# rrwick/Filtlong

Measured on AMD Instinct MI355X. Metric: Mbases/s scored+sorted, higher is better.
Workload: dtype f64; 1 GPU; 10,000,000 synthetic reads per GPU x gamma(k=4) mean 10 kbp, Phred-only, --target_bases 50008889515 (50% of bases); C2; reads_total=10000000, bases_total=100017779031, window_size=250, parallelism=1 GPU, device=AMD Radeon Graphics (gfx950:sramecc+:xnack-), gpus_visible=1, cut=select

## Files before the change

filtlong_amd/csrc/flx_ctx.hip:

```cpp
#include <algorithm>
#include <cmath>
#include <numeric>

#include "flx_internal.h"
#include <vector>

static std::string g_create_error;

int flx_fail(flx_ctx *ctx, int code, const char *fmt, ...) {
    char buf[1024];
    va_list ap;
    va_start(ap, fmt);
    vsnprintf(buf, sizeof buf, fmt, ap);
    va_end(ap);
    if (ctx) ctx->err = buf;
    else g_create_error = buf;
    return code;
}

extern "C" int flx_abi_version(void) { return FLX_ABI_VERSION; }

extern "C" int flx_device_count(void) {
    int n = 0;
    if (hipGetDeviceCount(&n) != hipSuccess) return -1;
// ... 84 lines not shown
}

extern "C" void flx_ctx_destroy(flx_ctx *ctx) {
    if (!ctx) return;
    (void)hipSetDevice(ctx->device);
    (void)hipStreamSynchronize(ctx->stream);
    (void)flx_comm_destroy(ctx);
    for (auto &t : ctx->timed) {
        (void)hipEventDestroy(t.start);
        (void)hipEventDestroy(t.stop);
    }
    for (auto ev : ctx->event_pool) (void)hipEventDestroy(ev);
    if (ctx->d_lut_q) (void)hipFree(ctx->d_lut_q);
    if (ctx->d_lut_d) (void)hipFree(ctx->d_lut_d);
    if (ctx->scratch) (void)hipFree(ctx->scratch);
    if (ctx->pinned) (void)hipHostFree(ctx->pinned);
    for (void *w : ctx->ws)
        if (w) (void)hipFree(w);
    if (ctx->own_stream) (void)hipStreamDestroy(ctx->own_stream);
    delete ctx;
}

extern "C" int flx_ctx_set_stream(flx_ctx *ctx, void *hip_stream) {
    if (!ctx) return FLX_ERR_INVALID;
    ctx->stream = hip_stream ? (hipStream_t)hip_stream : ctx->own_stream;
    return FLX_OK;
}

extern "C" int flx_ctx_synchronize(flx_ctx *ctx) {
    if (!ctx) return FLX_ERR_INVALID;
// ... 161 lines not shown
```

filtlong_amd/csrc/flx_internal.h:

```cpp
#pragma once

#include <hip/hip_runtime.h>

#include <cstdarg>
#include <cstdint>
#include <cstdio>
#include <cstdlib>
#include <cstring>
#include <string>
#include <vector>

#include "../../include/filtlong_hip.h"

struct flx_comm;

struct flx_timed_launch {
    const char *name;
    hipEvent_t start, stop;
};

struct flx_ctx {
    int device = 0;
    hipStream_t own_stream = nullptr;
    hipStream_t stream = nullptr;
    hipDeviceProp_t prop;
    std::string err;
    bool last_kmer_fold_grid = false;
    const uint8_t *last_kmer_redo = nullptr;
    uint64_t last_kmer_redo_n = 0;
    const char *last_kmer_cover = "";
    bool last_kmer_locus = false;
    void *phred_pending = nullptr;
    const char *last_phred_kernel = "";

    double h_lut_q[257];
    double *d_lut_q = nullptr;
    double *d_lut_d = nullptr;
    int lut_d_ws = -1;

    flx_comm *comm = nullptr;

    bool timing = false;
    std::vector<flx_timed_launch> timed;
    std::vector<size_t> timed_open;
    std::vector<hipEvent_t> event_pool;

    void *scratch = nullptr;
    size_t scratch_bytes = 0;
// ... 66 lines not shown
```

filtlong_amd/csrc/score_phred.hip:

```cpp
#include <algorithm>

#include "flx_internal.h"
#include "score_phred_common.h"

using namespace flx_phred;

namespace {

#ifndef FLX_CH
#define FLX_CH 64
#endif
constexpr int CH = FLX_CH;
constexpr int PPR = CH / 16;

struct Fold {
    double s;
    double w;
    double mn;
};

__device__ __forceinline__ void head16(const double *lq, const uint32_t (&lw)[4], Fold &f) {
    double qj[16];
#pragma unroll
    for (int i = 0; i < 16; ++i) qj[i] = lds_f64(lq, lut_addr(lw[i >> 2], i & 3));
// ... 320 lines not shown
    a.redo_list = nullptr;
    a.use_private = nullptr;
    a.long_thr = 0x7fffffff;

    const long long n_slots = ((long long)p->window_size + CH - 1) / CH + 1;
    long long slots16 = n_slots * CH / 16 + 1;
    if ((slots16 & 1) == 0) slots16 += 1;
    const size_t ring_bytes = (size_t)64 * slots16 * 16;

    int waves = (int)((kLdsBudget - kLutBytes) / ring_bytes);
    const char *env = getenv("FLX_PHRED_KERNEL");
    const bool force_direct = env && strcmp(env, "direct") == 0;
    const bool force_ring = env && strcmp(env, "ring") == 0;
    const bool force_stream = env && strcmp(env, "stream") == 0;
    const bool force_dual = env && strcmp(env, "dual") == 0;
    PhredLong lp;
    FLX_CHECK(flx_phred_long_detect(ctx, a, plane_bytes, &lp));
    if (force_stream || force_dual) {
        FLX_CHECK(flx_phred_long_split(ctx, a, &lp));
        if (a.n_reads == 0) return FLX_OK;
        return force_stream ? flx_launch_score_phred_stream(ctx, a) : flx_launch_score_phred_dual(ctx, a);
    }
    if (!force_direct && !force_ring) {
        bool launched = false;
        a.n_slots = 0;
        a.stride = 0;
        FLX_CHECK(flx_launch_score_phred_regs(ctx, a, &launched, &lp));
        if (launched) return FLX_OK;
        FLX_CHECK(flx_phred_long_split(ctx, a, &lp));
        if (a.n_reads == 0) return FLX_OK;
        return flx_launch_score_phred_dual(ctx, a);
    }
// ... 54 lines not shown
```

filtlong_amd/csrc/score_phred_common.h:

```cpp
#pragma once

#include "flx_internal.h"

namespace flx_phred {

constexpr int LUT_PAD = 264;

struct PhredArgs {
    const uint8_t *plane;
    const uint64_t *offsets;
    const int32_t *lengths;
    const uint32_t *order;
    uint64_t n_reads;
    const double *lut_q;
    const double *lut_d;
    int ws;
    int n_slots;
    int stride;
    double ws_d;
    double clamp;
    flx_params p;
    double *mean_q;
    double *window_q;
    uint8_t *passed;
    unsigned int *ticket;
    unsigned int n_groups;
    unsigned int *redo_count;
    uint32_t *redo_list;
    const unsigned int *use_private;
    int long_thr;
};

__device__ __forceinline__ int wave_max(int v) {
#pragma unroll
    for (int o = 32; o > 0; o >>= 1) v = max(v, __shfl_xor(v, o, 64));
    return __builtin_amdgcn_readfirstlane(v);
}
__device__ __forceinline__ int wave_min(int v) {
#pragma unroll
    for (int o = 32; o > 0; o >>= 1) v = min(v, __shfl_xor(v, o, 64));
    return __builtin_amdgcn_readfirstlane(v);
}

__device__ __forceinline__ uint32_t byte_of(const uint4 &v, int i) {
    const uint32_t d = (i >> 2) == 0 ? v.x : (i >> 2) == 1 ? v.y : (i >> 2) == 2 ? v.z : v.w;
// ... 28 lines not shown
__device__ __forceinline__ void finish_read(const PhredArgs &a, uint32_t rid, int L, double s, double mn) {
    const double mean = 100.0 * s / (double)L;
    double window;
    if (L <= a.ws) window = mean;
    else {
        if (mn < a.clamp) mn = 0.0;
        window = 100.0 * mn;
    }
    a.mean_q[rid] = mean;
    a.window_q[rid] = window;
    a.passed[rid] = hard_cutoffs(a.p, L, mean, window);
}

constexpr int PHRED_LONG_NB = 13;
constexpr long long PHRED_LONG_FLOOR = 1 << 18;
struct PhredLong {
    bool on = false;
    bool fetched = false;
    bool done = false;
    bool forced = false;
    int t0 = 0;
    uint64_t plane_bytes = 0;
    unsigned long long *d_counts = nullptr;
    unsigned long long h_counts[3 * PHRED_LONG_NB] = {};
};

}

int flx_phred_long_detect(flx_ctx *ctx, const flx_phred::PhredArgs &a, uint64_t plane_bytes, flx_phred::PhredLong *lp);
long long flx_phred_long_threshold(const flx_ctx *ctx, const flx_phred::PhredLong *lp, int *b0);
int flx_phred_long_fetch(flx_ctx *ctx, flx_phred::PhredLong *lp);
int flx_phred_long_split(flx_ctx *ctx, flx_phred::PhredArgs &a, flx_phred::PhredLong *lp);

int flx_launch_score_phred_regs(flx_ctx *ctx, flx_phred::PhredArgs a, bool *launched, flx_phred::PhredLong *lp);
int flx_launch_score_phred_stream(flx_ctx *ctx, flx_phred::PhredArgs a);
int flx_launch_score_phred_dual(flx_ctx *ctx, flx_phred::PhredArgs a);
```

filtlong_amd/csrc/score_phred_long.hip:

```cpp
#include <algorithm>
#include <cerrno>
#include <chrono>

#include "flx_internal.h"
#include "fold_map.h"
#include "score_phred_common.h"

using namespace flx_phred;
using namespace flx_fold;

namespace {

constexpr int LANE_EL = 16;
constexpr int CHUNK = 64 * LANE_EL;
constexpr long long SAT = 1ll << 61;
constexpr long long NOSTEP = 1ll << 62;
constexpr long long M_LO = (1ll << 52) + 1, M_HI = (1ll << 53) - 1;
constexpr int SLOT_BLOCKS = 1024;
constexpr int MAX_OPEN = 16;
constexpr int MAX_STALL = 2;
constexpr int MIN_ADVANCE = 4;

__device__ __forceinline__ long long sat(long long x) { return x > SAT ? SAT : x < -SAT ? -SAT : x; }
__device__ __forceinline__ long long sel(bool c, long long x1, long long x0) { return x0 ^ ((x0 ^ x1) & -(long long)c); }

__device__ __forceinline__ Map2 compose_sat(const Map2 &a, const Map2 &b) {
    Map2 c;
    c.a0 = sat(a.a0 + sel((a.a0 & 1) != 0, b.a1, b.a0));
    c.a1 = sat(a.a1 + sel(((1 + a.a1) & 1) != 0, b.a1, b.a0));
// ... 121 lines not shown
    if (pos >= L) return make_uint4(0, 0, 0, 0);
    return *reinterpret_cast<const uint4 *>(q + pos);
}

__global__ void __launch_bounds__(256) flx_score_phred_long_find(const int32_t *lengths, uint64_t n, int ws, int t0, int nb,
                                                                 unsigned long long *out) {
    __shared__ unsigned long long sh[3 * PHRED_LONG_NB];
    for (int i = threadIdx.x; i < 3 * PHRED_LONG_NB; i += 256) sh[i] = 0;
    __syncthreads();
    const uint64_t stride = (uint64_t)gridDim.x * 256;
    for (uint64_t i0 = (uint64_t)blockIdx.x * 256 + threadIdx.x; i0 < n; i0 += 4 * stride) {
        int Ls[4];
#pragma unroll
        for (int u = 0; u < 4; ++u) Ls[u] = i0 + u * stride < n ? lengths[i0 + u * stride] : 0;
#pragma unroll
        for (int u = 0; u < 4; ++u) {
            const int L = Ls[u];
            if (L >= t0) {
                int b = 0;
                if (nb > 1) b = min(nb - 1, (31 - __clz(L)) - (31 - __clz(t0)));
                atomicAdd(&sh[b], 1ull);
                atomicAdd(&sh[PHRED_LONG_NB + b], (unsigned long long)((L + CHUNK - 1) / CHUNK));
                if (L > ws) atomicAdd(&sh[2 * PHRED_LONG_NB + b], (unsigned long long)((L - ws + CHUNK - 1) / CHUNK));
            }
        }
    }
    __syncthreads();
    for (int i = threadIdx.x; i < 3 * PHRED_LONG_NB; i += 256)
        if (sh[i]) atomicAdd(&out[i], sh[i]);
}

__global__ void __launch_bounds__(256) flx_score_phred_long_count(const int32_t *lengths, const uint32_t *order, uint64_t n,
                                                                  uint64_t per, int thr, uint32_t *blk) {
    const uint64_t s0 = (uint64_t)blockIdx.x * per, s1 = min(n, s0 + per);
    int c = 0;
    for (uint64_t t = s0; t < s1; t += 256) {
        const uint64_t slot = t + threadIdx.x;
        bool f = false;
        if (slot < s1) f = lengths[order ? order[slot] : (uint32_t)slot] >= thr;
        c += __syncthreads_count(f);
// ... 446 lines not shown
                    }
                    opened += stalled >= MAX_STALL ? MAX_OPEN : 1;
                    ls = fl + 1;
                }
                cs = f + 1;
            }
        }
    }
    if (lane == 0) finish_read(g.a, rid, L, S, mn);
}

size_t up256(size_t x) { return (x + 255) & ~(size_t)255; }

}

int flx_phred_long_detect(flx_ctx *ctx, const PhredArgs &a, uint64_t plane_bytes, PhredLong *lp) {
    *lp = PhredLong();
    lp->plane_bytes = plane_bytes;
    long long t0 = PHRED_LONG_FLOOR;
    const char *env = getenv("FLX_PHRED_LONG_MIN");
    if (env) {
        char *end = nullptr;
        errno = 0;
        const unsigned long long v = strtoull(env, &end, 10);
        if (!*env || *end || errno || env[0] == '-' || env[0] == '+' || env[0] == ' ')
            return flx_fail(ctx, FLX_ERR_INVALID, "FLX_PHRED_LONG_MIN=%s: expected a non-negative integer (bases)", env);
        if (v == 0 || v > 0x7fffffffull) return FLX_OK;
        t0 = (long long)v;
        lp->forced = true;
    }
    void *w;
    FLX_CHECK(flx_workspace(ctx, 3, 4096, &w));
    lp->d_counts = (unsigned long long *)w;
    lp->t0 = (int)t0;
    FLX_HIP(ctx, hipMemsetAsync(w, 0, sizeof lp->h_counts, ctx->stream));
    const unsigned grid = (unsigned)std::min<uint64_t>((a.n_reads + 255) / 256, 2048);
    hipLaunchKernelGGL(flx_score_phred_long_find, dim3(grid), dim3(256), 0, ctx->stream, a.lengths, a.n_reads, a.ws, (int)t0,
                       lp->forced ? 1 : PHRED_LONG_NB, lp->d_counts);
    FLX_HIP(ctx, hipGetLastError());
    lp->on = true;
    return FLX_OK;
}

int flx_phred_long_fetch(flx_ctx *ctx, PhredLong *lp) {
    if (!lp || !lp->on || lp->fetched) return FLX_OK;
    FLX_HIP(ctx, hipMemcpyAsync(lp->h_counts, lp->d_counts, sizeof lp->h_counts, hipMemcpyDeviceToHost, ctx->stream));
    lp->fetched = true;
    return FLX_OK;
}
// ... 114 lines not shown
```

filtlong_amd/csrc/score_phred_regs.hip:

```cpp
#include <algorithm>

#include "flx_internal.h"
#include "score_phred_common.h"

using namespace flx_phred;

#ifndef FLX_REGS_PART
#define FLX_REGS_PART 0
#endif

namespace {

template <bool PRIV>
struct Tab {
    static constexpr int ROW = PRIV ? 256 : 8;
    static constexpr int ENTRIES = PRIV ? 129 : LUT_PAD;
    static constexpr int BYTES = ROW * ENTRIES;
    static constexpr int QOFF = 0;
    static constexpr int DOFF = BYTES;
    static constexpr int ZIDX = PRIV ? 128 : 256;
    static constexpr int SLOT0 = 2 * BYTES;
};

template <bool PRIV, int SEL>
// ... 66 lines not shown
}

__device__ __forceinline__ void funnel(const uint32_t (&p0)[4], const uint32_t (&p1)[4], int fD, uint32_t fsh, uint32_t (&tw)[4]) {
    const uint32_t x[8] = {p0[0], p0[1], p0[2], p0[3], p1[0], p1[1], p1[2], p1[3]};
#define FLX_FUN(D) _Pragma("unroll") for (int d = 0; d < 4; ++d) tw[d] = __builtin_amdgcn_alignbyte(x[(D) + d + 1], x[(D) + d], fsh);
    switch (fD) {
        case 0: FLX_FUN(0) break;
        case 1: FLX_FUN(1) break;
        case 2: FLX_FUN(2) break;
        case 3: FLX_FUN(3) break;
        default: tw[0] = x[4]; tw[1] = x[5]; tw[2] = x[6]; tw[3] = x[7]; break;
    }
#undef FLX_FUN
}

template <int A, bool PRIV, int WAVES>
__global__ void __launch_bounds__(WAVES * 64) flx_score_phred_regs(const PhredArgs a) {
    using T = Tab<PRIV>;
    if (a.use_private && (*a.use_private != 0u) != PRIV) return;
    constexpr int R = ((A + 5 + 3) / 4) * 4;
    constexpr int RR = R / 4;
    constexpr int H = (A + 1 + 3) / 4;
    constexpr int SLOT_BYTES = 8192;
    static_assert(H <= RR, "prologue must fit one ring revolution");
    extern __shared__ __attribute__((aligned(16))) unsigned char smem[];

    if (PRIV) {
        for (int i = threadIdx.x; i < 129 * 32; i += WAVES * 64) {
            const int e = i >> 5;
            const double q = e < 128 ? a.lut_q[e] : 0.0, d = e < 128 ? a.lut_d[e] : 0.0;
            *reinterpret_cast<double *>(smem + T::QOFF + i * 8) = q;
            *reinterpret_cast<double *>(smem + T::DOFF + i * 8) = d;
        }
    } else {
        for (int i = threadIdx.x; i < 257; i += WAVES * 64) {
            *reinterpret_cast<double *>(smem + T::QOFF + i * 8) = a.lut_q[i];
            *reinterpret_cast<double *>(smem + T::DOFF + i * 8) = a.lut_d[i];
        }
    }
    __syncthreads();

    const int lane = threadIdx.x & 63;
    const int wave = threadIdx.x >> 6;
    unsigned char *slot = smem + T::SLOT0 + wave * SLOT_BYTES;
    const uint32_t slot_lds = (uint32_t)__builtin_amdgcn_readfirstlane((int)(T::SLOT0 + wave * SLOT_BYTES));
    const unsigned char *my_row = slot + lane * 64;
    const int rot = lane >> 2;
    const uint32_t laneoff = (uint32_t)(lane & 31) * 8u;
    const uint32_t zaddr = PRIV ? (uint32_t)(T::ZIDX * T::ROW) + laneoff : (uint32_t)(T::ZIDX * T::ROW);
    const int ws = a.ws;
    const int B = ws & 15;
    const int fD = (16 - B) >> 2;
    const uint32_t fsh = (uint32_t)(16 - B) & 3u;
    const double ws_d = a.ws_d;

  for (;;) {
    unsigned int group = 0;
    if (lane == 0) group = atomicAdd(a.ticket, 1u);
// ... 148 lines not shown
#pragma unroll
            for (int k = 0; k < 4; ++k) {
                const int t = 4 * sr + k;
                const int Tp = 4 * r + k;
                if (16 * Tp >= Lmax) break;
                steady_piece(ring[t], ring[(t + R - A - 1) % R], ring[(t + R - A) % R], Tp);
            }
        }
    }
done:
    if (live) {
        finish_read(a, rid, L, s, mn);
        if (PRIV && (bad & 0x80808080u)) a.redo_list[atomicAdd(a.redo_count, 1u)] = rid;
    }
  }
}

#if FLX_REGS_PART == 0
__global__ void __launch_bounds__(1024) flx_score_phred_stream(const PhredArgs a) {
    using T = Tab<false>;
    extern __shared__ __attribute__((aligned(16))) unsigned char smem[];
    for (int i = threadIdx.x; i < 257; i += 1024) {
        *reinterpret_cast<double *>(smem + T::QOFF + i * 8) = a.lut_q[i];
        *reinterpret_cast<double *>(smem + T::DOFF + i * 8) = a.lut_d[i];
    }
    __syncthreads();
    const int lane = threadIdx.x & 63;
    const uint32_t zaddr = (uint32_t)(T::ZIDX * T::ROW);
    const int ws = a.ws;
    const int A = ws >> 4, B = ws & 15;
// ... 253 lines not shown
                            }
                        }
                    }
                }
            }
#pragma unroll
            for (int k = 0; k < 4; ++k) {
                prev[k][0] = cur[k][0]; prev[k][1] = cur[k][1]; prev[k][2] = cur[k][2]; prev[k][3] = cur[k][3];
            }
        }
        asm volatile("s_waitcnt vmcnt(0)" ::: "memory");
        if (live) finish_read(a, rid, L, s, mn);
    }
}

__global__ void __launch_bounds__(256) flx_score_phred_redo(const PhredArgs a) {
    __shared__ double lq[LUT_PAD];
    __shared__ double ld[LUT_PAD];
    for (int i = threadIdx.x; i < 257; i += 256) {
        lq[i] = a.lut_q[i];
        ld[i] = a.lut_d[i];
    }
    __syncthreads();
    const unsigned int n = *a.redo_count;
    for (unsigned int i = blockIdx.x * 256 + threadIdx.x; i < n; i += gridDim.x * 256) {
        const uint32_t rid = a.redo_list[i];
        const int L = a.lengths[rid];
        const uint8_t *q = a.plane + a.offsets[rid];
        const int ws = a.ws;
        double s = 0.0, w = 0.0, mn = 0.0;
        const int head = L < ws ? L : ws;
        for (int j = 0; j < head; ++j) s += lq[q[j]];
        if (L > ws) {
// ... 1 lines not shown
            mn = w;
            for (int j = ws; j < L; ++j) {
                const uint32_t cj = q[j], ci = q[j - ws];
                s += lq[cj];
                w -= ld[ci];
                w += ld[cj];
                if (w < mn) mn = w;
            }
        }
        finish_read(a, rid, L, s, mn);
    }
}

#endif

template <int A, bool PRIV, int WAVES>
int launch_one(flx_ctx *ctx, PhredArgs &a) {
    using T = Tab<PRIV>;
    auto kern = flx_score_phred_regs<A, PRIV, WAVES>;
    const size_t lds = std::max<size_t>((size_t)T::SLOT0 + (size_t)WAVES * 8192, 84 * 1024);
    FLX_HIP(ctx, hipFuncSetAttribute((const void *)kern, hipFuncAttributeMaxDynamicSharedMemorySize, (int)lds));
    const uint64_t per_block = (uint64_t)WAVES;
    const unsigned grid = (unsigned)std::min<uint64_t>(((uint64_t)a.n_groups + per_block - 1) / per_block,
                                                       (uint64_t)ctx->prop.multiProcessorCount);
    if (!a.use_private) {
        ctx->last_phred_kernel = PRIV ? "flx_score_phred_regs_private" : "flx_score_phred_regs";
        flx_time_begin(ctx, ctx->last_phred_kernel);
    }
    hipLaunchKernelGGL(kern, dim3(grid), dim3(WAVES * 64), lds, ctx->stream, a);
    if (!a.use_private) flx_time_end(ctx);
    FLX_HIP(ctx, hipGetLastError());
    return FLX_OK;
}

template <int A, bool PRIV>
struct WavesFor {
    static constexpr int plain = A <= 7 ? 16 : A <= 15 ? 12 : 8;
    static constexpr int value = PRIV && plain > 11 ? 11 : plain;
};

template <int A>
int launch_a(flx_ctx *ctx, PhredArgs &a, bool priv) {
    if constexpr (A >= 32) {
        return launch_one<A, false, WavesFor<A, false>::value>(ctx, a);
    } else {
        return priv ? launch_one<A, true, WavesFor<A, true>::value>(ctx, a) : launch_one<A, false, WavesFor<A, false>::value>(ctx, a);
    }
}

}

#define FLX_REGS_CASE(AA) \
    case AA:              \
        *launched = true; \
        return launch_a<AA>(ctx, a, priv);
#define FLX_REGS_CAT2(a, b) a##b
#define FLX_REGS_CAT(a, b) FLX_REGS_CAT2(a, b)
#define FLX_REGS_WIDE_NAME FLX_REGS_CAT(flx_launch_score_phred_regs_part, FLX_REGS_PART)
#if FLX_REGS_PART == 0
int flx_launch_score_phred_regs_part0(flx_ctx *ctx, PhredArgs &a, bool priv, bool *launched) {
    switch (a.ws / 16) { FLX_REGS_CASE(0) FLX_REGS_CASE(1) FLX_REGS_CASE(2) FLX_REGS_CASE(3) FLX_REGS_CASE(4) FLX_REGS_CASE(5) FLX_REGS_CASE(6) FLX_REGS_CASE(7) default: return FLX_OK; }
}
#elif FLX_REGS_PART == 1
int flx_launch_score_phred_regs_part1(flx_ctx *ctx, PhredArgs &a, bool priv, bool *launched) {
    switch (a.ws / 16) { FLX_REGS_CASE(8) FLX_REGS_CASE(9) FLX_REGS_CASE(10) FLX_REGS_CASE(11) FLX_REGS_CASE(12) default: return FLX_OK; }
}
#elif FLX_REGS_PART == 2
int flx_launch_score_phred_regs_part2(flx_ctx *ctx, PhredArgs &a, bool priv, bool *launched) {
    switch (a.ws / 16) { FLX_REGS_CASE(13) FLX_REGS_CASE(14) FLX_REGS_CASE(15) FLX_REGS_CASE(16) FLX_REGS_CASE(17) default: return FLX_OK; }
}
#elif FLX_REGS_PART == 3
int flx_launch_score_phred_regs_part3(flx_ctx *ctx, PhredArgs &a, bool priv, bool *launched) {
    switch (a.ws / 16) { FLX_REGS_CASE(18) FLX_REGS_CASE(19) FLX_REGS_CASE(20) FLX_REGS_CASE(21) FLX_REGS_CASE(22) default: return FLX_OK; }
}
#elif FLX_REGS_PART == 4
int flx_launch_score_phred_regs_part4(flx_ctx *ctx, PhredArgs &a, bool priv, bool *launched) {
    switch (a.ws / 16) { FLX_REGS_CASE(23) FLX_REGS_CASE(24) FLX_REGS_CASE(25) FLX_REGS_CASE(26) FLX_REGS_CASE(27) default: return FLX_OK; }
}
#elif FLX_REGS_PART == 5
int flx_launch_score_phred_regs_part5(flx_ctx *ctx, PhredArgs &a, bool priv, bool *launched) {
    switch (a.ws / 16) { FLX_REGS_CASE(28) FLX_REGS_CASE(29) FLX_REGS_CASE(30) FLX_REGS_CASE(31) default: return FLX_OK; }
}
#else
int FLX_REGS_WIDE_NAME(flx_ctx *ctx, PhredArgs &a, bool priv, bool *launched) {
    constexpr int A0 = 32 + 4 * (FLX_REGS_PART - 6);
    switch (a.ws / 16) {
        FLX_REGS_CASE(A0) FLX_REGS_CASE(A0 + 1) FLX_REGS_CASE(A0 + 2)
#if FLX_REGS_PART < 7
        FLX_REGS_CASE(A0 + 3)
#endif
        default: return FLX_OK;
    }
}
#endif
#undef FLX_REGS_CASE

#if FLX_REGS_PART == 0
int flx_launch_score_phred_regs_part1(flx_ctx *ctx, PhredArgs &a, bool priv, bool *launched);
int flx_launch_score_phred_regs_part2(flx_ctx *ctx, PhredArgs &a, bool priv, bool *launched);
int flx_launch_score_phred_regs_part3(flx_ctx *ctx, PhredArgs &a, bool priv, bool *launched);
int flx_launch_score_phred_regs_part4(flx_ctx *ctx, PhredArgs &a, bool priv, bool *launched);
int flx_launch_score_phred_regs_part5(flx_ctx *ctx, PhredArgs &a, bool priv, bool *launched);
#define FLX_REGS_DECL(P) int flx_launch_score_phred_regs_part##P(flx_ctx *ctx, PhredArgs &a, bool priv, bool *launched);
FLX_REGS_DECL(6) FLX_REGS_DECL(7)
#undef FLX_REGS_DECL

namespace {
__global__ void __launch_bounds__(256) flx_phred_sample(const PhredArgs a, unsigned int *hist, unsigned int *done, unsigned int *use_private) {
    const uint64_t t = (uint64_t)blockIdx.x * 256 + threadIdx.x;
    uint64_t z = (t + 1) * 0x9E3779B97F4A7C15ULL;
    z = (z ^ (z >> 30)) * 0xBF58476D1CE4E5B9ULL;
    z = (z ^ (z >> 27)) * 0x94D049BB133111EBULL;
    z ^= z >> 31;
    const uint64_t r = z % a.n_reads;
    const int L = a.lengths[r];
    if (L > 0) {
        const uint32_t pos = (uint32_t)((z >> 32) % (uint64_t)L);
        atomicAdd(&hist[a.plane[a.offsets[r] + pos]], 1u);
    }
    __threadfence();
    __syncthreads();
    if (threadIdx.x != 0 || atomicAdd(done, 1u) != gridDim.x - 1) return;
    __threadfence();
    double tot = 0.0, conflicts = 0.0;
    bool high = false;
    for (int i = 0; i < 256; ++i) {
        const unsigned int h = __hip_atomic_load(&hist[i], __ATOMIC_RELAXED, __HIP_MEMORY_SCOPE_AGENT);
        tot += h;
        high = high || (i >= 128 && h != 0);
    }
    if (tot > 0) {
        for (int b = 0; b < 32; ++b) {
            double pb = 0.0, sq = 0.0;
            for (int e = b; e < 256; e += 32) {
                const double pe = __hip_atomic_load(&hist[e], __ATOMIC_RELAXED, __HIP_MEMORY_SCOPE_AGENT) / tot;
                pb += pe;
                sq += pe * pe;
            }
            conflicts += pb * pb - sq;
        }
    }
    *use_private = (!high && 496.0 * conflicts > 3.0) ? 1u : 0u;
}

struct PhredPending {
    PhredArgs a;
    PhredLong lp;
    bool chosen_on_device;
    long timed_index;
    const unsigned int *h_flag;
    const unsigned long long *h_counts;
};
}

int flx_launch_score_phred_stream(flx_ctx *ctx, PhredArgs a) {
    void *scr;
    FLX_CHECK(flx_scratch(ctx, 64, &scr));
// ... 23 lines not shown
    flx_time_begin(ctx, ctx->last_phred_kernel);
#define FLX_DUAL_LAUNCH(M)                                                                                                              \
    case M:                                                                                                                             \
        FLX_HIP(ctx, hipFuncSetAttribute((const void *)flx_score_phred_dual<M>, hipFuncAttributeMaxDynamicSharedMemorySize, (int)lds)); \
        hipLaunchKernelGGL(flx_score_phred_dual<M>, dim3(grid), dim3(DUAL_WAVES * 64), lds, ctx->stream, a);                            \
        break;
    switch ((a.ws >> 4) & 3) {
        FLX_DUAL_LAUNCH(0) FLX_DUAL_LAUNCH(1) FLX_DUAL_LAUNCH(2) FLX_DUAL_LAUNCH(3)
    }
#undef FLX_DUAL_LAUNCH
    flx_time_end(ctx);
    FLX_HIP(ctx, hipGetLastError());
    return FLX_OK;
}

int flx_launch_score_phred_regs(flx_ctx *ctx, PhredArgs a, bool *launched, PhredLong *lp) {
    *launched = false;
    const int A = a.ws / 16;
    if (A > 38) return FLX_OK;
    const char *env = getenv("FLX_PHRED_TABLES");
    bool priv = env && strcmp(env, "private") == 0;
    bool forced = env && (strcmp(env, "private") == 0 || strcmp(env, "plain") == 0);
    if (A >= 32) {
        forced = true;
        priv = false;
    }
    delete (PhredPending *)ctx->phred_pending;
    ctx->phred_pending = nullptr;
    void *scr;
    FLX_CHECK(flx_scratch(ctx, 2048 + a.n_reads * 4, &scr));
    void *pin;
    FLX_CHECK(flx_pinned(ctx, 1024, &pin));
    a.ticket = (unsigned int *)scr;
    a.redo_count = (unsigned int *)scr + 1;
    a.redo_list = (uint32_t *)((char *)scr + 2048);
    unsigned int *d_flag = (unsigned int *)scr + 3;
    FLX_HIP(ctx, hipMemsetAsync(scr, 0, 2048, ctx->stream));
    if (!forced) {
        hipLaunchKernelGGL(flx_phred_sample, dim3(64), dim3(256), 0, ctx->stream, a, (unsigned int *)((char *)scr + 64),
                           (unsigned int *)scr + 2, d_flag);
        a.use_private = d_flag;
    }
    a.long_thr = (int)std::min<long long>(flx_phred_long_threshold(ctx, lp, nullptr), 0x7fffffff);
    a.n_groups = (unsigned int)((a.n_reads + 63) / 64);
    auto part = [&](bool pv) -> int {
        if (A <= 7) return flx_launch_score_phred_regs_part0(ctx, a, pv, launched);
        if (A <= 12) return flx_launch_score_phred_regs_part1(ctx, a, pv, launched);
        if (A <= 17) return flx_launch_score_phred_regs_part2(ctx, a, pv, launched);
        if (A <= 22) return flx_launch_score_phred_regs_part3(ctx, a, pv, launched);
        if (A <= 27) return flx_launch_score_phred_regs_part4(ctx, a, pv, launched);
        if (A <= 31) return flx_launch_score_phred_regs_part5(ctx, a, pv, launched);
        typedef int (*part_fn)(flx_ctx *, PhredArgs &, bool, bool *);
        static const part_fn wide[2] = {flx_launch_score_phred_regs_part6, flx_launch_score_phred_regs_part7};
        return wide[(A - 32) / 4](ctx, a, false, launched);
    };
    long timed_index = -1;
    if (forced) {
        FLX_CHECK(part(priv));
    } else {
        ctx->last_phred_kernel = "flx_score_phred_regs";
        flx_time_scope t(ctx, ctx->last_phred_kernel);
        if (ctx->timing) timed_index = (long)ctx->timed.size() - 1;
        FLX_CHECK(part(false));
        FLX_CHECK(part(true));
    }
    if (!*launched) return FLX_OK;
    if (priv || !forced) {
        flx_time_begin(ctx, "flx_score_phred_redo");
        hipLaunchKernelGGL(flx_score_phred_redo, dim3(256), dim3(256), 0, ctx->stream, a);
        flx_time_end(ctx);
        FLX_HIP(ctx, hipGetLastError());
    }
    PhredPending *pd = new PhredPending();
    pd->a = a;
    pd->lp = *lp;
    pd->chosen_on_device = !forced;
    pd->timed_index = timed_index;
    pd->h_flag = (const unsigned int *)pin;
    pd->h_counts = (const unsigned long long *)((char *)pin + 64);
    ctx->phred_pending = pd;
    if (!forced) FLX_HIP(ctx, hipMemcpyAsync(pin, d_flag, 4, hipMemcpyDeviceToHost, ctx->stream));
    if (lp->on) FLX_HIP(ctx, hipMemcpyAsync((char *)pin + 64, lp->d_counts, sizeof lp->h_counts, hipMemcpyDeviceToHost, ctx->stream));
    lp->done = true;
    return FLX_OK;
}

int flx_phred_finish(flx_ctx *ctx) {
    PhredPending *pd = (PhredPending *)ctx->phred_pending;
    if (!pd) return FLX_OK;
    ctx->phred_pending = nullptr;
    struct Free {
        PhredPending *p;
        ~Free() { delete p; }
    } guard{pd};
    if (pd->chosen_on_device) {
        ctx->last_phred_kernel = *pd->h_flag ? "flx_score_phred_regs_private" : "flx_score_phred_regs";
        if (pd->timed_index >= 0 && (size_t)pd->timed_index < ctx->timed.size()) ctx->timed[pd->timed_index].name = ctx->last_phred_kernel;
// ... 13 lines not shown
```

Measured before the change: 3.331 million Mbases/s.

## Fuse phred sample and long-read detection into one prepare kernel, single regs launch

Merges the long-read length histogram and the table-conflict sampling into one prepare kernel. A persistent device state block, reset by the redo kernel, replaces the per-call memset. The plain and private score kernels, previously launched back to back with one exiting early, become a single kernel that branches on the device-side flag, and the sample's final reduction is parallelised. This removes several small launches and memsets per scoring call, at the cost of a wider block shape for the private variant and more template complexity.

```diff
diff --git a/filtlong_amd/csrc/flx_ctx.hip b/filtlong_amd/csrc/flx_ctx.hip
--- a/filtlong_amd/csrc/flx_ctx.hip
+++ b/filtlong_amd/csrc/flx_ctx.hip
@@ -122,6 +122,7 @@
     if (ctx->d_lut_q) (void)hipFree(ctx->d_lut_q);
     if (ctx->d_lut_d) (void)hipFree(ctx->d_lut_d);
     if (ctx->scratch) (void)hipFree(ctx->scratch);
+    if (ctx->phred_state) (void)hipFree(ctx->phred_state);
     if (ctx->pinned) (void)hipHostFree(ctx->pinned);
     for (void *w : ctx->ws)
         if (w) (void)hipFree(w);
diff --git a/filtlong_amd/csrc/flx_internal.h b/filtlong_amd/csrc/flx_internal.h
--- a/filtlong_amd/csrc/flx_internal.h
+++ b/filtlong_amd/csrc/flx_internal.h
@@ -32,6 +32,9 @@
     bool last_kmer_locus = false;
     void *phred_pending = nullptr;
     const char *last_phred_kernel = "";
+    void *phred_state = nullptr;
+    bool phred_state_clean = false;
+    hipStream_t phred_state_stream = nullptr;
 
     double h_lut_q[257];
     double *d_lut_q = nullptr;
diff --git a/filtlong_amd/csrc/score_phred.hip b/filtlong_amd/csrc/score_phred.hip
--- a/filtlong_amd/csrc/score_phred.hip
+++ b/filtlong_amd/csrc/score_phred.hip
@@ -358,8 +358,9 @@
     const bool force_ring = env && strcmp(env, "ring") == 0;
     const bool force_stream = env && strcmp(env, "stream") == 0;
     const bool force_dual = env && strcmp(env, "dual") == 0;
+    const bool regs_path = !force_stream && !force_dual && !force_direct && !force_ring && flx_phred_regs_serves(p->window_size);
     PhredLong lp;
-    FLX_CHECK(flx_phred_long_detect(ctx, a, plane_bytes, &lp));
+    FLX_CHECK(flx_phred_long_detect(ctx, a, plane_bytes, &lp, !regs_path));
     if (force_stream || force_dual) {
         FLX_CHECK(flx_phred_long_split(ctx, a, &lp));
         if (a.n_reads == 0) return FLX_OK;
diff --git a/filtlong_amd/csrc/score_phred_common.h b/filtlong_amd/csrc/score_phred_common.h
--- a/filtlong_amd/csrc/score_phred_common.h
+++ b/filtlong_amd/csrc/score_phred_common.h
@@ -28,7 +28,18 @@
     unsigned int *redo_count;
     uint32_t *redo_list;
     const unsigned int *use_private;
+    int force_private;
     int long_thr;
+};
+
+struct PhredState {
+    unsigned int ticket;
+    unsigned int redo_count;
+    unsigned int sample_done;
+    unsigned int use_private;
+    unsigned int pad[12];
+    unsigned int hist[256];
+    unsigned long long long_counts[3 * 13];
 };
 
 __device__ __forceinline__ int wave_max(int v) {
@@ -87,6 +98,18 @@
 
 constexpr int PHRED_LONG_NB = 13;
 constexpr long long PHRED_LONG_FLOOR = 1 << 18;
+constexpr int PHRED_LONG_CHUNK = 1024;
+static_assert(sizeof(PhredState::long_counts) == 3 * PHRED_LONG_NB * sizeof(unsigned long long), "PhredState holds the detection's counts");
+
+__device__ __forceinline__ void phred_long_count(int L, int ws, int t0, int nb, unsigned long long *sh) {
+    if (L < t0) return;
+    int b = 0;
+    if (nb > 1) b = min(nb - 1, (31 - __clz(L)) - (31 - __clz(t0)));
+    atomicAdd(&sh[b], 1ull);
+    atomicAdd(&sh[PHRED_LONG_NB + b], (unsigned long long)((L + PHRED_LONG_CHUNK - 1) / PHRED_LONG_CHUNK));
+    if (L > ws) atomicAdd(&sh[2 * PHRED_LONG_NB + b], (unsigned long long)((L - ws + PHRED_LONG_CHUNK - 1) / PHRED_LONG_CHUNK));
+}
+
 struct PhredLong {
     bool on = false;
     bool fetched = false;
@@ -100,11 +123,13 @@
 
 }
 
-int flx_phred_long_detect(flx_ctx *ctx, const flx_phred::PhredArgs &a, uint64_t plane_bytes, flx_phred::PhredLong *lp);
+int flx_phred_long_detect(flx_ctx *ctx, const flx_phred::PhredArgs &a, uint64_t plane_bytes, flx_phred::PhredLong *lp,
+                          bool count_now = true);
 long long flx_phred_long_threshold(const flx_ctx *ctx, const flx_phred::PhredLong *lp, int *b0);
 int flx_phred_long_fetch(flx_ctx *ctx, flx_phred::PhredLong *lp);
 int flx_phred_long_split(flx_ctx *ctx, flx_phred::PhredArgs &a, flx_phred::PhredLong *lp);
 
+bool flx_phred_regs_serves(int window_size);
 int flx_launch_score_phred_regs(flx_ctx *ctx, flx_phred::PhredArgs a, bool *launched, flx_phred::PhredLong *lp);
 int flx_launch_score_phred_stream(flx_ctx *ctx, flx_phred::PhredArgs a);
 int flx_launch_score_phred_dual(flx_ctx *ctx, flx_phred::PhredArgs a);
diff --git a/filtlong_amd/csrc/score_phred_long.hip b/filtlong_amd/csrc/score_phred_long.hip
--- a/filtlong_amd/csrc/score_phred_long.hip
+++ b/filtlong_amd/csrc/score_phred_long.hip
@@ -13,6 +13,7 @@
 
 constexpr int LANE_EL = 16;
 constexpr int CHUNK = 64 * LANE_EL;
+static_assert(CHUNK == PHRED_LONG_CHUNK, "the detection counts chunks of this size");
 constexpr long long SAT = 1ll << 61;
 constexpr long long NOSTEP = 1ll << 62;
 constexpr long long M_LO = (1ll << 52) + 1, M_HI = (1ll << 53) - 1;
@@ -164,16 +165,7 @@
 #pragma unroll
         for (int u = 0; u < 4; ++u) Ls[u] = i0 + u * stride < n ? lengths[i0 + u * stride] : 0;
 #pragma unroll
-        for (int u = 0; u < 4; ++u) {
-            const int L = Ls[u];
-            if (L >= t0) {
-                int b = 0;
-                if (nb > 1) b = min(nb - 1, (31 - __clz(L)) - (31 - __clz(t0)));
-                atomicAdd(&sh[b], 1ull);
-                atomicAdd(&sh[PHRED_LONG_NB + b], (unsigned long long)((L + CHUNK - 1) / CHUNK));
-                if (L > ws) atomicAdd(&sh[2 * PHRED_LONG_NB + b], (unsigned long long)((L - ws + CHUNK - 1) / CHUNK));
-            }
-        }
+        for (int u = 0; u < 4; ++u) phred_long_count(Ls[u], ws, t0, nb, sh);
     }
     __syncthreads();
     for (int i = threadIdx.x; i < 3 * PHRED_LONG_NB; i += 256)
@@ -650,7 +642,7 @@
 
 }
 
-int flx_phred_long_detect(flx_ctx *ctx, const PhredArgs &a, uint64_t plane_bytes, PhredLong *lp) {
+int flx_phred_long_detect(flx_ctx *ctx, const PhredArgs &a, uint64_t plane_bytes, PhredLong *lp, bool count_now) {
     *lp = PhredLong();
     lp->plane_bytes = plane_bytes;
     long long t0 = PHRED_LONG_FLOOR;
@@ -665,10 +657,14 @@
         t0 = (long long)v;
         lp->forced = true;
     }
+    lp->t0 = (int)t0;
+    if (!count_now) {
+        lp->on = true;
+        return FLX_OK;
+    }
     void *w;
     FLX_CHECK(flx_workspace(ctx, 3, 4096, &w));
     lp->d_counts = (unsigned long long *)w;
-    lp->t0 = (int)t0;
     FLX_HIP(ctx, hipMemsetAsync(w, 0, sizeof lp->h_counts, ctx->stream));
     const unsigned grid = (unsigned)std::min<uint64_t>((a.n_reads + 255) / 256, 2048);
     hipLaunchKernelGGL(flx_score_phred_long_find, dim3(grid), dim3(256), 0, ctx->stream, a.lengths, a.n_reads, a.ws, (int)t0,
diff --git a/filtlong_amd/csrc/score_phred_regs.hip b/filtlong_amd/csrc/score_phred_regs.hip
--- a/filtlong_amd/csrc/score_phred_regs.hip
+++ b/filtlong_amd/csrc/score_phred_regs.hip
@@ -104,10 +104,10 @@
 #undef FLX_FUN
 }
 
-template <int A, bool PRIV, int WAVES>
-__global__ void __launch_bounds__(WAVES * 64) flx_score_phred_regs(const PhredArgs a) {
+template <int A, bool PRIV, int WAVES, int BLOCK_WAVES>
+__device__ __forceinline__ void phred_regs_body(const PhredArgs &a) {
     using T = Tab<PRIV>;
-    if (a.use_private && (*a.use_private != 0u) != PRIV) return;
+    static_assert(WAVES <= BLOCK_WAVES, "a slot per scoring wave");
     constexpr int R = ((A + 5 + 3) / 4) * 4;
     constexpr int RR = R / 4;
     constexpr int H = (A + 1 + 3) / 4;
@@ -116,14 +116,14 @@
     extern __shared__ __attribute__((aligned(16))) unsigned char smem[];
 
     if (PRIV) {
-        for (int i = threadIdx.x; i < 129 * 32; i += WAVES * 64) {
+        for (int i = threadIdx.x; i < 129 * 32; i += BLOCK_WAVES * 64) {
             const int e = i >> 5;
             const double q = e < 128 ? a.lut_q[e] : 0.0, d = e < 128 ? a.lut_d[e] : 0.0;
             *reinterpret_cast<double *>(smem + T::QOFF + i * 8) = q;
             *reinterpret_cast<double *>(smem + T::DOFF + i * 8) = d;
         }
     } else {
-        for (int i = threadIdx.x; i < 257; i += WAVES * 64) {
+        for (int i = threadIdx.x; i < 257; i += BLOCK_WAVES * 64) {
             *reinterpret_cast<double *>(smem + T::QOFF + i * 8) = a.lut_q[i];
             *reinterpret_cast<double *>(smem + T::DOFF + i * 8) = a.lut_d[i];
         }
@@ -132,6 +132,7 @@
 
     const int lane = threadIdx.x & 63;
     const int wave = threadIdx.x >> 6;
+    if (WAVES < BLOCK_WAVES && wave >= WAVES) return;
     unsigned char *slot = smem + T::SLOT0 + wave * SLOT_BYTES;
     const uint32_t slot_lds = (uint32_t)__builtin_amdgcn_readfirstlane((int)(T::SLOT0 + wave * SLOT_BYTES));
     const unsigned char *my_row = slot + lane * 64;
@@ -310,6 +311,25 @@
         if (PRIV && (bad & 0x80808080u)) a.redo_list[atomicAdd(a.redo_count, 1u)] = rid;
     }
   }
+}
+
+template <int A, bool PRIV>
+struct WavesFor {
+    static constexpr int plain = A <= 7 ? 16 : A <= 15 ? 12 : 8;
+    static constexpr int value = PRIV && plain > 11 ? 11 : plain;
+};
+
+template <int A, bool BOTH>
+__global__ void __launch_bounds__((WavesFor<A, false>::value * 64)) flx_score_phred_regs(const PhredArgs a) {
+    constexpr int BW = WavesFor<A, false>::value;
+    if constexpr (BOTH) {
+        const bool priv = a.use_private ? *a.use_private != 0u : a.force_private != 0;
+        if (priv) {
+            phred_regs_body<A, true, WavesFor<A, true>::value, BW>(a);
+            return;
+        }
+    }
+    phred_regs_body<A, false, BW, BW>(a);
 }
 
 #if FLX_REGS_PART == 0
@@ -593,9 +613,14 @@
     }
 }
 
-__global__ void __launch_bounds__(256) flx_score_phred_redo(const PhredArgs a) {
+__global__ void __launch_bounds__(256) flx_score_phred_redo(const PhredArgs a, PhredState *st) {
     __shared__ double lq[LUT_PAD];
     __shared__ double ld[LUT_PAD];
+    if (blockIdx.x == 0) {
+        st->hist[threadIdx.x] = 0u;
+        if (threadIdx.x < 3 * PHRED_LONG_NB) st->long_counts[threadIdx.x] = 0ull;
+        if (threadIdx.x == 0) st->sample_done = 0u;
+    }
     for (int i = threadIdx.x; i < 257; i += 256) {
         lq[i] = a.lut_q[i];
         ld[i] = a.lut_d[i];
@@ -627,38 +652,21 @@
 
 #endif
 
-template <int A, bool PRIV, int WAVES>
-int launch_one(flx_ctx *ctx, PhredArgs &a) {
-    using T = Tab<PRIV>;
-    auto kern = flx_score_phred_regs<A, PRIV, WAVES>;
-    const size_t lds = std::max<size_t>((size_t)T::SLOT0 + (size_t)WAVES * 8192, 84 * 1024);
+template <int A>
+int launch_a(flx_ctx *ctx, PhredArgs &a) {
+    constexpr bool BOTH = A < 32;
+    constexpr int BW = WavesFor<A, false>::value;
+    auto kern = flx_score_phred_regs<A, BOTH>;
+    size_t lds = std::max<size_t>((size_t)Tab<false>::SLOT0 + (size_t)BW * 8192, 84 * 1024);
+    if (BOTH) lds = std::max<size_t>(lds, (size_t)Tab<true>::SLOT0 + (size_t)WavesFor<A, true>::value * 8192);
+    static_assert((size_t)Tab<true>::SLOT0 + 11 * 8192 <= 160 * 1024, "the bank-private tables and 11 slots fit the LDS");
     FLX_HIP(ctx, hipFuncSetAttribute((const void *)kern, hipFuncAttributeMaxDynamicSharedMemorySize, (int)lds));
-    const uint64_t per_block = (uint64_t)WAVES;
+    const uint64_t per_block = (uint64_t)BW;
     const unsigned grid = (unsigned)std::min<uint64_t>(((uint64_t)a.n_groups + per_block - 1) / per_block,
                                                        (uint64_t)ctx->prop.multiProcessorCount);
-    if (!a.use_private) {
-        ctx->last_phred_kernel = PRIV ? "flx_score_phred_regs_private" : "flx_score_phred_regs";
-        flx_time_begin(ctx, ctx->last_phred_kernel);
-    }
-    hipLaunchKernelGGL(kern, dim3(grid), dim3(WAVES * 64), lds, ctx->stream, a);
-    if (!a.use_private) flx_time_end(ctx);
+    hipLaunchKernelGGL(kern, dim3(grid), dim3(BW * 64), lds, ctx->stream, a);
     FLX_HIP(ctx, hipGetLastError());
     return FLX_OK;
-}
-
-template <int A, bool PRIV>
-struct WavesFor {
-    static constexpr int plain = A <= 7 ? 16 : A <= 15 ? 12 : 8;
-    static constexpr int value = PRIV && plain > 11 ? 11 : plain;
-};
-
-template <int A>
-int launch_a(flx_ctx *ctx, PhredArgs &a, bool priv) {
-    if constexpr (A >= 32) {
-        return launch_one<A, false, WavesFor<A, false>::value>(ctx, a);
-    } else {
-        return priv ? launch_one<A, true, WavesFor<A, true>::value>(ctx, a) : launch_one<A, false, WavesFor<A, false>::value>(ctx, a);
-    }
 }
 
 }
@@ -666,36 +674,36 @@
 #define FLX_REGS_CASE(AA) \
     case AA:              \
         *launched = true; \
-        return launch_a<AA>(ctx, a, priv);
+        return launch_a<AA>(ctx, a);
 #define FLX_REGS_CAT2(a, b) a##b
 #define FLX_REGS_CAT(a, b) FLX_REGS_CAT2(a, b)
 #define FLX_REGS_WIDE_NAME FLX_REGS_CAT(flx_launch_score_phred_regs_part, FLX_REGS_PART)
 #if FLX_REGS_PART == 0
-int flx_launch_score_phred_regs_part0(flx_ctx *ctx, PhredArgs &a, bool priv, bool *launched) {
+int flx_launch_score_phred_regs_part0(flx_ctx *ctx, PhredArgs &a, bool *launched) {
     switch (a.ws / 16) { FLX_REGS_CASE(0) FLX_REGS_CASE(1) FLX_REGS_CASE(2) FLX_REGS_CASE(3) FLX_REGS_CASE(4) FLX_REGS_CASE(5) FLX_REGS_CASE(6) FLX_REGS_CASE(7) default: return FLX_OK; }
 }
 #elif FLX_REGS_PART == 1
-int flx_launch_score_phred_regs_part1(flx_ctx *ctx, PhredArgs &a, bool priv, bool *launched) {
+int flx_launch_score_phred_regs_part1(flx_ctx *ctx, PhredArgs &a, bool *launched) {
     switch (a.ws / 16) { FLX_REGS_CASE(8) FLX_REGS_CASE(9) FLX_REGS_CASE(10) FLX_REGS_CASE(11) FLX_REGS_CASE(12) default: return FLX_OK; }
 }
 #elif FLX_REGS_PART == 2
-int flx_launch_score_phred_regs_part2(flx_ctx *ctx, PhredArgs &a, bool priv, bool *launched) {
+int flx_launch_score_phred_regs_part2(flx_ctx *ctx, PhredArgs &a, bool *launched) {
     switch (a.ws / 16) { FLX_REGS_CASE(13) FLX_REGS_CASE(14) FLX_REGS_CASE(15) FLX_REGS_CASE(16) FLX_REGS_CASE(17) default: return FLX_OK; }
 }
 #elif FLX_REGS_PART == 3
-int flx_launch_score_phred_regs_part3(flx_ctx *ctx, PhredArgs &a, bool priv, bool *launched) {
+int flx_launch_score_phred_regs_part3(flx_ctx *ctx, PhredArgs &a, bool *launched) {
     switch (a.ws / 16) { FLX_REGS_CASE(18) FLX_REGS_CASE(19) FLX_REGS_CASE(20) FLX_REGS_CASE(21) FLX_REGS_CASE(22) default: return FLX_OK; }
 }
 #elif FLX_REGS_PART == 4
-int flx_launch_score_phred_regs_part4(flx_ctx *ctx, PhredArgs &a, bool priv, bool *launched) {
+int flx_launch_score_phred_regs_part4(flx_ctx *ctx, PhredArgs &a, bool *launched) {
     switch (a.ws / 16) { FLX_REGS_CASE(23) FLX_REGS_CASE(24) FLX_REGS_CASE(25) FLX_REGS_CASE(26) FLX_REGS_CASE(27) default: return FLX_OK; }
 }
 #elif FLX_REGS_PART == 5
-int flx_launch_score_phred_regs_part5(flx_ctx *ctx, PhredArgs &a, bool priv, bool *launched) {
+int flx_launch_score_phred_regs_part5(flx_ctx *ctx, PhredArgs &a, bool *launched) {
     switch (a.ws / 16) { FLX_REGS_CASE(28) FLX_REGS_CASE(29) FLX_REGS_CASE(30) FLX_REGS_CASE(31) default: return FLX_OK; }
 }
 #else
-int FLX_REGS_WIDE_NAME(flx_ctx *ctx, PhredArgs &a, bool priv, bool *launched) {
+int FLX_REGS_WIDE_NAME(flx_ctx *ctx, PhredArgs &a, bool *launched) {
     constexpr int A0 = 32 + 4 * (FLX_REGS_PART - 6);
     switch (a.ws / 16) {
         FLX_REGS_CASE(A0) FLX_REGS_CASE(A0 + 1) FLX_REGS_CASE(A0 + 2)
@@ -709,17 +717,42 @@
 #undef FLX_REGS_CASE
 
 #if FLX_REGS_PART == 0
-int flx_launch_score_phred_regs_part1(flx_ctx *ctx, PhredArgs &a, bool priv, bool *launched);
-int flx_launch_score_phred_regs_part2(flx_ctx *ctx, PhredArgs &a, bool priv, bool *launched);
-int flx_launch_score_phred_regs_part3(flx_ctx *ctx, PhredArgs &a, bool priv, bool *launched);
-int flx_launch_score_phred_regs_part4(flx_ctx *ctx, PhredArgs &a, bool priv, bool *launched);
-int flx_launch_score_phred_regs_part5(flx_ctx *ctx, PhredArgs &a, bool priv, bool *launched);
-#define FLX_REGS_DECL(P) int flx_launch_score_phred_regs_part##P(flx_ctx *ctx, PhredArgs &a, bool priv, bool *launched);
+int flx_launch_score_phred_regs_part1(flx_ctx *ctx, PhredArgs &a, bool *launched);
+int flx_launch_score_phred_regs_part2(flx_ctx *ctx, PhredArgs &a, bool *launched);
+int flx_launch_score_phred_regs_part3(flx_ctx *ctx, PhredArgs &a, bool *launched);
+int flx_launch_score_phred_regs_part4(flx_ctx *ctx, PhredArgs &a, bool *launched);
+int flx_launch_score_phred_regs_part5(flx_ctx *ctx, PhredArgs &a, bool *launched);
+#define FLX_REGS_DECL(P) int flx_launch_score_phred_regs_part##P(flx_ctx *ctx, PhredArgs &a, bool *launched);
 FLX_REGS_DECL(6) FLX_REGS_DECL(7)
 #undef FLX_REGS_DECL
 
 namespace {
-__global__ void __launch_bounds__(256) flx_phred_sample(const PhredArgs a, unsigned int *hist, unsigned int *done, unsigned int *use_private) {
+constexpr int SAMPLE_WGS = 64;
+__global__ void __launch_bounds__(256) flx_phred_prepare(const PhredArgs a, PhredState *st, int do_sample, int long_t0, int long_nb) {
+    __shared__ unsigned long long sh[3 * PHRED_LONG_NB];
+    __shared__ unsigned int h[256];
+    __shared__ double cb[32];
+    __shared__ unsigned int last;
+    if (blockIdx.x == 0 && threadIdx.x == 0) {
+        st->ticket = 0u;
+        st->redo_count = 0u;
+    }
+    if (long_nb > 0) {
+        for (int i = threadIdx.x; i < 3 * PHRED_LONG_NB; i += 256) sh[i] = 0;
+        __syncthreads();
+        const uint64_t n = a.n_reads, stride = (uint64_t)gridDim.x * 256;
+        for (uint64_t i0 = (uint64_t)blockIdx.x * 256 + threadIdx.x; i0 < n; i0 += 4 * stride) {
+            int Ls[4];
+#pragma unroll
+            for (int u = 0; u < 4; ++u) Ls[u] = i0 + u * stride < n ? a.lengths[i0 + u * stride] : 0;
+#pragma unroll
+            for (int u = 0; u < 4; ++u) phred_long_count(Ls[u], a.ws, long_t0, long_nb, sh);
+        }
+        __syncthreads();
+        for (int i = threadIdx.x; i < 3 * PHRED_LONG_NB; i += 256)
+            if (sh[i]) atomicAdd(&st->long_counts[i], sh[i]);
+    }
+    if (!do_sample || blockIdx.x >= SAMPLE_WGS) return;
     const uint64_t t = (uint64_t)blockIdx.x * 256 + threadIdx.x;
     uint64_t z = (t + 1) * 0x9E3779B97F4A7C15ULL;
     z = (z ^ (z >> 30)) * 0xBF58476D1CE4E5B9ULL;
@@ -729,31 +762,34 @@
     const int L = a.lengths[r];
     if (L > 0) {
         const uint32_t pos = (uint32_t)((z >> 32) % (uint64_t)L);
-        atomicAdd(&hist[a.plane[a.offsets[r] + pos]], 1u);
+        atomicAdd(&st->hist[a.plane[a.offsets[r] + pos]], 1u);
     }
     __threadfence();
     __syncthreads();
-    if (threadIdx.x != 0 || atomicAdd(done, 1u) != gridDim.x - 1) return;
+    if (threadIdx.x == 0) last = atomicAdd(&st->sample_done, 1u) == SAMPLE_WGS - 1 ? 1u : 0u;
+    __syncthreads();
+    if (!last) return;
     __threadfence();
-    double tot = 0.0, conflicts = 0.0;
-    bool high = false;
-    for (int i = 0; i < 256; ++i) {
-        const unsigned int h = __hip_atomic_load(&hist[i], __ATOMIC_RELAXED, __HIP_MEMORY_SCOPE_AGENT);
-        tot += h;
-        high = high || (i >= 128 && h != 0);
-    }
-    if (tot > 0) {
-        for (int b = 0; b < 32; ++b) {
-            double pb = 0.0, sq = 0.0;
-            for (int e = b; e < 256; e += 32) {
-                const double pe = __hip_atomic_load(&hist[e], __ATOMIC_RELAXED, __HIP_MEMORY_SCOPE_AGENT) / tot;
+    h[threadIdx.x] = __hip_atomic_load(&st->hist[threadIdx.x], __ATOMIC_RELAXED, __HIP_MEMORY_SCOPE_AGENT);
+    const int high = __syncthreads_or(threadIdx.x >= 128 && h[threadIdx.x] != 0);
+    if (threadIdx.x < 32) {
+        double tot = 0.0;
+        for (int i = 0; i < 256; ++i) tot += h[i];
+        double pb = 0.0, sq = 0.0;
+        if (tot > 0) {
+            for (int e = threadIdx.x; e < 256; e += 32) {
+                const double pe = h[e] / tot;
                 pb += pe;
                 sq += pe * pe;
             }
-            conflicts += pb * pb - sq;
-        }
-    }
-    *use_private = (!high && 496.0 * conflicts > 3.0) ? 1u : 0u;
+        }
+        cb[threadIdx.x] = pb * pb - sq;
+    }
+    __syncthreads();
+    if (threadIdx.x != 0) return;
+    double conflicts = 0.0;
+    for (int b = 0; b < 32; ++b) conflicts += cb[b];
+    st->use_private = (!high && 496.0 * conflicts > 3.0) ? 1u : 0u;
 }
 
 struct PhredPending {
@@ -807,10 +843,12 @@
     return FLX_OK;
 }
 
+bool flx_phred_regs_serves(int window_size) { return window_size / 16 <= 38; }
+
 int flx_launch_score_phred_regs(flx_ctx *ctx, PhredArgs a, bool *launched, PhredLong *lp) {
     *launched = false;
     const int A = a.ws / 16;
-    if (A > 38) return FLX_OK;
+    if (!flx_phred_regs_serves(a.ws)) return FLX_OK;
     const char *env = getenv("FLX_PHRED_TABLES");
     bool priv = env && strcmp(env, "private") == 0;
     bool forced = env && (strcmp(env, "private") == 0 || strcmp(env, "plain") == 0);
@@ -820,50 +858,48 @@
     }
     delete (PhredPending *)ctx->phred_pending;
     ctx->phred_pending = nullptr;
+    if (!ctx->phred_state) {
+        FLX_HIP(ctx, hipMalloc(&ctx->phred_state, sizeof(PhredState)));
+        ctx->phred_state_clean = false;
+    }
+    PhredState *st = (PhredState *)ctx->phred_state;
+    if (!ctx->phred_state_clean || ctx->phred_state_stream != ctx->stream)
+        FLX_HIP(ctx, hipMemsetAsync(st, 0, sizeof(PhredState), ctx->stream));
+    ctx->phred_state_clean = false;
+    ctx->phred_state_stream = ctx->stream;
     void *scr;
-    FLX_CHECK(flx_scratch(ctx, 2048 + a.n_reads * 4, &scr));
+    FLX_CHECK(flx_scratch(ctx, 256 + a.n_reads * 4, &scr));
     void *pin;
     FLX_CHECK(flx_pinned(ctx, 1024, &pin));
-    a.ticket = (unsigned int *)scr;
-    a.redo_count = (unsigned int *)scr + 1;
-    a.redo_list = (uint32_t *)((char *)scr + 2048);
-    unsigned int *d_flag = (unsigned int *)scr + 3;
-    FLX_HIP(ctx, hipMemsetAsync(scr, 0, 2048, ctx->stream));
-    if (!forced) {
-        hipLaunchKernelGGL(flx_phred_sample, dim3(64), dim3(256), 0, ctx->stream, a, (unsigned int *)((char *)scr + 64),
-                           (unsigned int *)scr + 2, d_flag);
-        a.use_private = d_flag;
-    }
+    a.ticket = &st->ticket;
+    a.redo_count = &st->redo_count;
+    a.redo_list = (uint32_t *)scr;
+    a.use_private = forced ? nullptr : &st->use_private;
+    a.force_private = priv ? 1 : 0;
     a.long_thr = (int)std::min<long long>(flx_phred_long_threshold(ctx, lp, nullptr), 0x7fffffff);
     a.n_groups = (unsigned int)((a.n_reads + 63) / 64);
-    auto part = [&](bool pv) -> int {
-        if (A <= 7) return flx_launch_score_phred_regs_part0(ctx, a, pv, launched);
-        if (A <= 12) return flx_launch_score_phred_regs_part1(ctx, a, pv, launched);
-        if (A <= 17) return flx_launch_score_phred_regs_part2(ctx, a, pv, launched);
-        if (A <= 22) return flx_launch_score_phred_regs_part3(ctx, a, pv, launched);
-        if (A <= 27) return flx_launch_score_phred_regs_part4(ctx, a, pv, launched);
-        if (A <= 31) return flx_launch_score_phred_regs_part5(ctx, a, pv, launched);
-        typedef int (*part_fn)(flx_ctx *, PhredArgs &, bool, bool *);
-        static const part_fn wide[2] = {flx_launch_score_phred_regs_part6, flx_launch_score_phred_regs_part7};
-        return wide[(A - 32) / 4](ctx, a, false, launched);
-    };
+    if (lp->on) lp->d_counts = st->long_counts;
+    {
+        const unsigned grid = lp->on ? (unsigned)std::max<uint64_t>(SAMPLE_WGS, std::min<uint64_t>((a.n_reads + 255) / 256, 2048)) : SAMPLE_WGS;
+        hipLaunchKernelGGL(flx_phred_prepare, dim3(grid), dim3(256), 0, ctx->stream, a, st, forced ? 0 : 1, lp->t0,
+                           lp->on ? (lp->forced ? 1 : PHRED_LONG_NB) : 0);
+        FLX_HIP(ctx, hipGetLastError());
+    }
     long timed_index = -1;
-    if (forced) {
-        FLX_CHECK(part(priv));
-    } else {
-        ctx->last_phred_kernel = "flx_score_phred_regs";
+    {
+        ctx->last_phred_kernel = priv ? "flx_score_phred_regs_private" : "flx_score_phred_regs";
         flx_time_scope t(ctx, ctx->last_phred_kernel);
         if (ctx->timing) timed_index = (long)ctx->timed.size() - 1;
-        FLX_CHECK(part(false));
-        FLX_CHECK(part(true));
-    }
-    if (!*launched) return FLX_OK;
-    if (priv || !forced) {
-        flx_time_begin(ctx, "flx_score_phred_redo");
-        hipLaunchKernelGGL(flx_score_phred_redo, dim3(256), dim3(256), 0, ctx->stream, a);
-        flx_time_end(ctx);
-        FLX_HIP(ctx, hipGetLastError());
-    }
+        if (A <= 7) FLX_CHECK(flx_launch_score_phred_regs_part0(ctx, a, launched));
+        else if (A <= 12) FLX_CHECK(flx_launch_score_phred_regs_part1(ctx, a, launched));
+        else if (A <= 17) FLX_CHECK(flx_launch_score_phred_regs_part2(ctx, a, launched));
+        else if (A <= 22) FLX_CHECK(flx_launch_score_phred_regs_part3(ctx, a, launched));
+        else if (A <= 27) FLX_CHECK(flx_launch_score_phred_regs_part4(ctx, a, launched));
+        else if (A <= 31) FLX_CHECK(flx_launch_score_phred_regs_part5(ctx, a, launched));
+        else if (A <= 35) FLX_CHECK(flx_launch_score_phred_regs_part6(ctx, a, launched));
+        else FLX_CHECK(flx_launch_score_phred_regs_part7(ctx, a, launched));
+    }
+    if (!*launched) return flx_fail(ctx, FLX_ERR_STATE, "no register-history kernel for window size %d", a.ws);
     PhredPending *pd = new PhredPending();
     pd->a = a;
     pd->lp = *lp;
@@ -872,8 +908,13 @@
     pd->h_flag = (const unsigned int *)pin;
     pd->h_counts = (const unsigned long long *)((char *)pin + 64);
     ctx->phred_pending = pd;
-    if (!forced) FLX_HIP(ctx, hipMemcpyAsync(pin, d_flag, 4, hipMemcpyDeviceToHost, ctx->stream));
+    if (!forced) FLX_HIP(ctx, hipMemcpyAsync(pin, &st->use_private, 4, hipMemcpyDeviceToHost, ctx->stream));
     if (lp->on) FLX_HIP(ctx, hipMemcpyAsync((char *)pin + 64, lp->d_counts, sizeof lp->h_counts, hipMemcpyDeviceToHost, ctx->stream));
+    flx_time_begin(ctx, "flx_score_phred_redo");
+    hipLaunchKernelGGL(flx_score_phred_redo, dim3(priv || !forced ? 256 : 1), dim3(256), 0, ctx->stream, a, st);
+    flx_time_end(ctx);
+    FLX_HIP(ctx, hipGetLastError());
+    ctx->phred_state_clean = true;
     lp->done = true;
     return FLX_OK;
 }
```

After: 3.336 million Mbases/s, median of 6. No clear change (+0.2%).
